# JuliaParallel/DistributedArrays.jl

Measured on NVIDIA H100. Metric: GB/s for map! and sum on Float32 DArray, higher is better.
Workload: dtype f32

## Files before the change

distributedarrays.jl_b200/_broadcast.py:

```python
from __future__ import annotations

import ctypes as C
import struct
from typing import Callable, List, Optional, Sequence, Tuple

import numpy as np

from builtins import any as builtins_any

from . import _lib
from ._darray import B200Array, DArray, dab_dtype, darray, makelocal
from .layout import shape_of
from .runtime import close_remote_reads, open_remote_reads, runtime

_RANK = {"bool": 0, "i32": 1, "i64": 2, "i128": 3, "f32": 4, "f64": 5}


class _TagTypes(dict):

    def __missing__(self, tag):
        raise _lib.UnsupportedError(_lib.ERR_UNSUPPORTED, f"values of type {tag} have no array element type on the GPU backend "
                                    "(Int128 is served as the value type of mapreduce(f, op, d) only)")


_NPT = _TagTypes({"bool": np.dtype(np.bool_), "i32": np.dtype(np.int32), "i64": np.dtype(np.int64), "f32": np.dtype(np.float32),
                  "f64": np.dtype(np.float64), "c64": np.dtype(np.complex64), "c128": np.dtype(np.complex128)})
# ... 426 lines not shown


def jl_max(a, b):
    return binop("max", Expr.wrap(a), Expr.wrap(b))


def jl_min(a, b):
    return binop("min", Expr.wrap(a), Expr.wrap(b))


def mod(a, b):
    return binop("mod", Expr.wrap(a), Expr.wrap(b))


def rem(a, b):
    return binop("rem", Expr.wrap(a), Expr.wrap(b))


def trace(f: Callable, arg_tags: Sequence[str]) -> Expr:
    syms = [Expr("arg", (), t, k) for k, t in enumerate(arg_tags)]
    return Expr.wrap(f(*syms))


_FN2 = {"add": "jl_add", "sub": "jl_sub", "mul": "jl_mul", "div": "jl_div", "rem": "jl_rem", "mod": "jl_mod", "idiv": "jl_idiv",
        "max": "jl_max", "min": "jl_min", "pow": "jl_pow", "and": "jl_and", "or": "jl_or", "xor": "jl_xor", "lt": "jl_lt", "le": "jl_le",
        "gt": "jl_gt", "ge": "jl_ge", "eq": "jl_eq", "ne": "jl_ne", "x_shl": "jl_x_shl", "x_shr": "jl_x_shr"}
_FN2.update({"m_copysign": "jl_m_copysign", "m_powi": "jl_m_powi"})
_FN2.update({"m_" + c: "jl_m_" + c for c in ("lt", "le", "gt", "ge", "eq", "ne")})


def _lit(jt: str, v) -> str:
    if jt == "f32":
        return "__int_as_float((int)0x%08x)" % struct.unpack("<I", struct.pack("<f", float(v)))[0]
    if jt == "f64":
        return "__longlong_as_double((long long)0x%016xULL)" % struct.unpack("<Q", struct.pack("<d", float(v)))[0]
    if is_ctag(jt):
        z = complex(v)
        return "%s(%s, %s)" % (_CT[jt], _lit(_COMP[jt], z.real), _lit(_COMP[jt], z.imag))
    if jt == "i32":
        return "((int)%d)" % int(v)
    if jt == "i64":
        return "((long long)%dLL)" % int(v)
    if jt == "i128":
        v = int(v) % (1 << 128)
        return "((i128)(((u128)0x%016xULL << 64) | (u128)0x%016xULL))" % (v >> 64, v & ((1 << 64) - 1))
    return "true" if v else "false"
# ... 75 lines not shown
        groups.append((o, ext))
    if not groups:
        groups = [(1, [1] * len(shapes))]
    return tuple(g[0] for g in groups), [tuple(g[1][k] for g in groups) for k in range(len(shapes))]


def _dense_strides(shape):
    s, out = 1, []
    for d in shape:
        out.append(s)
        s *= int(d)
    return out


class LocalArg:

    def __init__(self, arr: Optional[B200Array] = None, scalar=None, tag: str = "f64", temp: bool = False):
        self.arr, self.scalar, self.tag, self.temp = arr, scalar, tag, temp


def run_local(rt, expr: Expr, out: B200Array, largs: List[LocalArg]):
    n = out.size
    if n == 0:
        return
    out_tag = tag_of(out.dtype)
    full = [a for a in largs if a.arr is not None]
    same = all(a.arr.shape == out.shape or a.arr.size == n and _squeeze(a.arr.shape) == _squeeze(out.shape) for a in full)
    ctx = rt.ctx
    code = dab_dtype(out.dtype)
    rt.last_kernel = "fixed"
    cplx = uses_complex(expr) or builtins_any(is_ctag(a.tag) for a in largs)
    if same and not cplx and expr.jt == out_tag and out_tag != "bool":
        x0 = largs[0] if largs and largs[0].arr is not None and largs[0].tag == out_tag else None
        if x0 is not None and all(_only_arg0(expr)):
            ab = match_affine(expr)
            if ab is not None:
                a = np.asarray(ab[0], dtype=out.dtype)
                b = np.asarray(ab[1], dtype=out.dtype)
                _lib.call("dab_affine", ctx, code, C.c_void_p(out.ptr), C.c_void_p(x0.arr.ptr), C.c_void_p(a.ctypes.data),
                          C.c_void_p(b.ctypes.data), n)
                rt.last_kernel = "dab_affine"
                return
            if expr.op in _UN and _is_arg(expr.args[0], 0):
                _lib.call("dab_unary", ctx, code, _UN[expr.op], C.c_void_p(out.ptr), C.c_void_p(x0.arr.ptr), n)
                return
            if _is_arg(expr, 0):
                _lib.call("dab_unary", ctx, code, _lib.MAP_ID, C.c_void_p(out.ptr), C.c_void_p(x0.arr.ptr), n)
                return
        if expr.op in _BIN and len(expr.args) == 2 and not (expr.op == "div" and out_tag[0] != "f"):
            l, r = expr.args
            la = largs[l.val] if l.op == "arg" else None
            ra = largs[r.val] if r.op == "arg" else None

            def arr_ok(e, a):
                return e.op == "arg" and a is not None and a.arr is not None and a.tag == out_tag

            def sc_val(e, a):
                if e.op == "const" and e.jt == out_tag:
                    return e.val
                if e.op == "arg" and a is not None and a.arr is None and a.tag == out_tag:
                    return a.scalar
                return None

            if arr_ok(l, la) and arr_ok(r, ra):
                _lib.call("dab_binary", ctx, code, _BIN[expr.op], C.c_void_p(out.ptr), C.c_void_p(la.arr.ptr), C.c_void_p(ra.arr.ptr), n)
# ... 120 lines not shown
            out.append((lo, hi))
        else:
            out.append((1, s))
    return tuple(out)


def _localise(rt, a, I, pid) -> LocalArg:
    if isinstance(a, DArray):
        view = _bcview(a.dims, I)
        arr = makelocal(a, view, pid)
        return LocalArg(arr, None, tag_of(a.dtype), temp=arr is not a.chunks.get(pid))
    if isinstance(a, np.ndarray) and a.ndim > 0:
        view = _bcview(a.shape, I)
        sl = a[tuple(slice(lo - 1, hi) for lo, hi in view)]
        return LocalArg(B200Array.from_numpy(rt, sl), None, tag_of(a.dtype), temp=True)
    e = Expr.wrap(a.item() if isinstance(a, np.ndarray) else a)
    return LocalArg(None, e.val, e.jt)


def _remote_args(dest_layout, args) -> List[DArray]:
    return [a for a in args if isinstance(a, DArray) and not (a.layout.pids == dest_layout.pids and a.layout.indices == dest_layout.indices)]


def _broadcast_chunks(dest: DArray, expr: Expr, args) -> DArray:
    rt = dest.rt
    fenced = open_remote_reads(rt, _remote_args(dest.layout, args), "host")
    for pid, out in dest.chunks.items():
        I = dest.layout.localindices(pid)
        largs = [_localise(rt, a, I, pid) for a in args]
        run_local(rt, expr, out, largs)
        for la in largs:
            if la.temp and la.arr is not None:
                la.arr.free()
    close_remote_reads(rt, fenced, "host")
    return dest


def _materialise_views(args):
    from ._darray import SubDArray
    out, temps = [], []
    for a in args:
        if isinstance(a, SubDArray):
            a = a.to_darray()
            temps.append(a)
        out.append(a)
    return out, temps


def broadcast_into(dest: DArray, f: Callable, *args) -> DArray:
    args, _views = _materialise_views(args)
    try:
        return _broadcast_into(dest, f, *args)
    finally:
        for v in _views:
            v.close()


def _broadcast_into(dest: DArray, f: Callable, *args) -> DArray:
    shapes = [a.dims if isinstance(a, DArray) else (a.shape if isinstance(a, np.ndarray) else ()) for a in args]
    for shp in shapes:
        for k, s in enumerate(shp):
            want = dest.dims[k] if k < len(dest.dims) else 1
            if s != 1 and s != want:
                raise _lib.DimensionMismatch(_lib.ERR_DIM_MISMATCH, f"destination axes {dest.dims} are not compatible with source axes {tuple(shp)}")
    expr = trace(f, [_arg_tag(a) for a in args])
    return _broadcast_chunks(dest, expr, args)


def broadcast(f: Callable, *args, rt=None) -> DArray:
    args, _views = _materialise_views(args)
    try:
        return _broadcast(f, *args, rt=rt)
    finally:
        for v in _views:
            v.close()


def _broadcast(f: Callable, *args, rt=None) -> DArray:
    rt = rt or next((a.rt for a in args if isinstance(a, DArray)), None) or runtime()
    shapes = [a.dims if isinstance(a, DArray) else (a.shape if isinstance(a, np.ndarray) else ()) for a in args]
    dims = _bc_shape(shapes)
    expr = trace(f, [_arg_tag(a) for a in args])
    out_dt = _NPT[expr.jt]
    dest = darray(lambda I: B200Array.empty(rt, shape_of(I), out_dt), dims, dtype=out_dt, rt=rt)
    return _broadcast_chunks(dest, expr, args)


def copy(d: DArray) -> DArray:
    from ._darray import similar
    return _broadcast_into(similar(d), lambda x: x, d)


deepcopy = copy


def drandn(dims, procs=None, dist=None, dtype=np.float64, seed: int = 1234, rt=None) -> DArray:
    from ._darray import component_dtype, drand
    dt = np.dtype(dtype)
    if dt.kind == "c":
        ct = component_dtype(dt)
        re = drandn(dims, procs, dist, dtype=ct, seed=seed, rt=rt)
        im = drandn(dims, procs, dist, dtype=ct, seed=seed + 2, rt=rt)
        from ._darray import darray_like
        out = darray_like(lambda I: B200Array.empty(re.rt, shape_of(I), dt), re, dtype=dt)
        _broadcast_into(out, lambda a, b: complex_(0.7071067811865476 * a, 0.7071067811865476 * b), re, im)
# ... 55 lines not shown
```

distributedarrays.jl_b200/_darray.py:

```python
from __future__ import annotations

import ctypes as C
import itertools
import weakref
from typing import Callable, Dict, List, Optional, Sequence, Tuple

import numpy as np

from . import _lib
from .layout import Layout, Range, default_procs, layout_from_chunk_shapes, make_layout, rlen, shape_of, slab_plan
from .runtime import Runtime, close_remote_reads, open_remote_reads, runtime

_DT = {np.dtype(np.float32): _lib.F32, np.dtype(np.float64): _lib.F64, np.dtype(np.int32): _lib.I32,
       np.dtype(np.int64): _lib.I64, np.dtype(np.bool_): _lib.U8,
       np.dtype(np.complex64): _lib.C64, np.dtype(np.complex128): _lib.C128}
_NP = {_lib.F32: np.dtype(np.float32), _lib.F64: np.dtype(np.float64), _lib.I32: np.dtype(np.int32),
       _lib.I64: np.dtype(np.int64), _lib.U8: np.dtype(np.bool_), _lib.C64: np.dtype(np.complex64), _lib.C128: np.dtype(np.complex128)}


def dab_dtype(dt) -> int:
    dt = np.dtype(dt)
    if dt not in _DT:
        raise _lib.UnsupportedError(_lib.ERR_UNSUPPORTED, f"element type {dt} is not served by the GPU backend (no host fallback)")
    return _DT[dt]


# ... 22 lines not shown
    __slots__ = ("rt", "ptr", "shape", "dtype", "_own", "_keep", "_temp")

    def __init__(self, rt: Runtime, ptr: int, shape: Sequence[int], dtype, own: bool = True, keep=None, temp: bool = False):
        self.rt, self.ptr, self.shape, self.dtype = rt, int(ptr), tuple(int(s) for s in shape), np.dtype(dtype)
        self._own, self._keep, self._temp = own, keep, temp

    @classmethod
    def empty(cls, rt: Runtime, shape: Sequence[int], dtype, temp: bool = False) -> "B200Array":
        dtype = np.dtype(dtype)
        n = int(np.prod(shape)) if len(shape) else 1
        ptr = rt.alloc_temp(n * dtype.itemsize) if temp else rt.alloc(n * dtype.itemsize)
        return cls(rt, ptr, shape, dtype, temp=temp)

    @classmethod
    def from_numpy(cls, rt: Runtime, a: np.ndarray) -> "B200Array":
        a = np.asarray(a)
        dab_dtype(a.dtype)
        out = cls.empty(rt, a.shape, a.dtype)
        out.copy_from_host(a)
        return out

    @property
    def size(self) -> int:
        return int(np.prod(self.shape)) if len(self.shape) else 1

    @property
    def nbytes(self) -> int:
        return self.size * self.dtype.itemsize

    @property
    def ndim(self) -> int:
        return len(self.shape)

    def copy_from_host(self, a: np.ndarray, sync: bool = True):
        a = np.asarray(a, dtype=self.dtype)
        if tuple(a.shape) != self.shape:
            raise _lib.DimensionMismatch(_lib.ERR_DIM_MISMATCH, f"host array {a.shape} vs chunk {self.shape}")
        if self.size == 0:
            return
        if not a.flags.f_contiguous:
            if a.ndim == 2 and a.strides[0] == a.itemsize and a.strides[1] > 0:
                _lib.call("dab_h2d_2d", self.rt.ctx, C.c_void_p(self.ptr), a.shape[0] * a.itemsize, C.c_void_p(a.ctypes.data),
                          a.strides[1], a.shape[0] * a.itemsize, a.shape[1])
                if sync:
                    self.rt.sync()
                return
            a = np.asfortranarray(a)
# ... 657 lines not shown
```

distributedarrays.jl_b200/_mapreduce.py:

```python
from __future__ import annotations

import builtins
import ctypes as C
import operator
from typing import Callable, Dict, Optional, Sequence, Tuple

import numpy as np

from . import _lib
from ._broadcast import Expr, broadcast, is_ctag, tag_of, trace, _NPT
from ._darray import B200Array, DArray, component_dtype, dab_dtype, is_complex, np_dtype
from .layout import Layout, collapse_for_region, ravel, shape_of, unravel
from .runtime import close_remote_reads, exchange_stacks, fence, grouped_exchange, open_remote_reads

_OPS = {"+": _lib.SUM, "add": _lib.SUM, "sum": _lib.SUM, "*": _lib.PROD, "mul": _lib.PROD, "prod": _lib.PROD, "max": _lib.MAX,
        "min": _lib.MIN}
_OPF = {operator.add: _lib.SUM, operator.mul: _lib.PROD, builtins.max: _lib.MAX, builtins.min: _lib.MIN, np.add: _lib.SUM,
        np.multiply: _lib.PROD, np.maximum: _lib.MAX, np.minimum: _lib.MIN}


def _op_code(op) -> int:
    if isinstance(op, str) and op in _OPS:
        return _OPS[op]
    if op in _OPF:
        return _OPF[op]
    raise _lib.UnsupportedError(_lib.ERR_UNSUPPORTED, f"reduction operator {op!r} is not served by a kernel (no host fallback)")
# ... 25 lines not shown
    if e.op in _CMPMAP:
        l, r = e.args

        def unpromote(side, const):
            if side.op == "convert" and side.args[0].op == "arg" and side.args[0].jt == tag and const.op == "const":
                c = const.val
                if tag == "f32" and const.jt == "f64" and float(np.float32(c)) == c:
                    return side.args[0], Expr("const", (), tag, c)
                if tag in ("i32", "i64") and const.jt in ("i64",) and side.jt == "i64":
                    return side.args[0], Expr("const", (), tag, c) if -2**31 <= c < 2**31 or tag == "i64" else (side, const)
            return side, const

        l, r = unpromote(l, r)
        r, l = unpromote(r, l)
        if l.op == "arg" and r.op == "const" and l.jt == tag:
            return _CMPMAP[e.op], np.asarray(r.val, dtype=np.dtype(dtype)), e
        if r.op == "arg" and l.op == "const" and r.jt == tag:
            return _CMPMAP[_FLIP[e.op]], np.asarray(l.val, dtype=np.dtype(dtype)), e
    if e.op == "isnan" and e.args[0].op == "arg":
        return _lib.MAP_ISNAN, None, e
    return None, None, e


def _result_dtype(dtype, op: int, mapc: int) -> np.dtype:
    out = C.c_int32()
    _lib.check(_lib.lib().dab_reduce_result_dtype(dab_dtype(dtype), op, mapc, C.byref(out)))
    return np.dtype(np.int64) if out.value == _lib.I64 else np_dtype(out.value)




def _gather_slots(d: DArray, launch: Callable[[int, B200Array, int], None]) -> np.ndarray:
    rt = d.rt
    wpr = rt.workers_per_rank
    slots = B200Array.empty(rt, (16 * wpr,), np.uint8, temp=True)
    try:
        for pid, ch in d.chunks.items():
            launch(pid, ch, slots.ptr + 16 * ((pid - 1) % wpr))
        if rt.world > 1:
            allslots = B200Array.empty(rt, (16 * wpr * rt.world,), np.uint8, temp=True)
            _lib.call("dab_allgather", rt.ctx, C.c_void_p(slots.ptr), C.c_void_p(allslots.ptr), 16 * wpr)
            host = allslots.to_numpy()
            allslots.free()
        else:
            host = slots.to_numpy()
    finally:
# ... 109 lines not shown
    return (res, vals) if return_partials else res


def _mapreduce_all(f, op, d: DArray, return_partials: bool = False, others: Sequence = ()):
    opc = op if isinstance(op, int) else _op_code(op)
    if others:
        expr = trace(f, [tag_of(d.dtype)] + [_arg_tag_of(a) for a in others])
        return _mapreduce_expr(expr, opc, d, others, return_partials)
    mapc, param, expr = classify_map(f, d.dtype)
    if is_complex(d.dtype) and mapc is not None and not _complex_served(opc, mapc):
        if mapc == _lib.MAP_ID and opc in (_lib.MAX, _lib.MIN):
            raise TypeError(f"MethodError: no method matching isless(::{d.dtype}, ::{d.dtype}) -- complex numbers are not ordered")
        mapc = None
        if expr is None:
            expr = trace(lambda z: z, [tag_of(d.dtype)])
    if mapc is None:
        return _mapreduce_expr(expr, opc, d, (), return_partials)
    _check_nonempty(d, opc)
    rt = d.rt
    pp = C.c_void_p(param.ctypes.data) if param is not None else None
    rdt = _result_dtype(d.dtype, opc, mapc)
    if rt.workers_per_rank == 1 and d.layout.pids == rt.workers() and not return_partials:
        ch = d.chunks[rt.myid()]
        out = np.zeros(2, dtype=np.uint64)
        _lib.call("dab_mapreduce_all", rt.ctx, dab_dtype(d.dtype), opc, mapc, pp, C.c_void_p(ch.ptr), ch.size, C.c_void_p(out.ctypes.data))
        return out.view(np.uint8)[:rdt.itemsize].view(rdt)[0]
    code = dab_dtype(d.dtype)
    host = _gather_slots(d, lambda pid, ch, slot: _lib.call("dab_reduce", rt.ctx, code, opc, mapc, pp, C.c_void_p(ch.ptr), ch.size, C.c_void_p(slot)))
    res, vals = _fold(host, d.layout.pids, rdt, opc)
    return (res, vals) if return_partials else res


def _complex_served(opc: int, mapc: int) -> bool:
    out = C.c_int32()
    return _lib.lib().dab_reduce_result_dtype(_lib.C64, opc, mapc, C.byref(out)) == _lib.OK


def _arg_tag_of(a) -> str:
    from ._broadcast import _arg_tag
    return _arg_tag(a)


def reduce(op, d: DArray, dims=None, init=None):
    return mapreduce(None, op, d, dims=dims, init=init)


def mapreduce(f: Optional[Callable], op, d: DArray, *ds, dims=None, init=None, _partials: bool = False):
    from ._darray import SubDArray
    if isinstance(d, Expr):
# ... 403 lines not shown
```

distributedarrays.jl_b200/csrc/dab_comm.cu:

```cuda
#include <dlfcn.h>
#include <nccl.h>

#include "dab_common.cuh"
#include "dab_scalar_ops.cuh"

namespace {

struct NcclApi {
    void* handle = nullptr;
    ncclResult_t (*GetUniqueId)(ncclUniqueId*) = nullptr;
    ncclResult_t (*CommInitRank)(ncclComm_t*, int, ncclUniqueId, int) = nullptr;
    ncclResult_t (*CommDestroy)(ncclComm_t) = nullptr;
    ncclResult_t (*AllGather)(const void*, void*, size_t, ncclDataType_t, ncclComm_t, cudaStream_t) = nullptr;
    ncclResult_t (*AllReduce)(const void*, void*, size_t, ncclDataType_t, ncclRedOp_t, ncclComm_t, cudaStream_t) = nullptr;
    ncclResult_t (*Send)(const void*, size_t, ncclDataType_t, int, ncclComm_t, cudaStream_t) = nullptr;
    ncclResult_t (*Recv)(void*, size_t, ncclDataType_t, int, ncclComm_t, cudaStream_t) = nullptr;
    ncclResult_t (*GroupStart)() = nullptr;
    ncclResult_t (*GroupEnd)() = nullptr;
    const char* (*GetErrorString)(ncclResult_t) = nullptr;
    const char* (*GetLastError)(ncclComm_t) = nullptr;
    bool ok = false;
    char why[256] = "";
};

// ... 67 lines not shown
    while (*mine < seq) {
        if ((++spins & 1023u) == 0 && dab_globaltimer_ns() - t0 > timeout_ns) {
            host_status[0] = 1ull;
            __threadfence_system();
            break;
        }
    }
    __threadfence_system();
}

template <typename T>
__global__ void __launch_bounds__(256) accumulate_stack_kernel(T* __restrict__ y, size_t n, T beta, int beta_mode, T alpha, int alpha_one,
                                                              const T* __restrict__ stack, size_t stride, int count) {
    for (size_t i = (size_t)blockIdx.x * 256 + threadIdx.x; i < n; i += (size_t)gridDim.x * 256) {
        T v = beta_mode == 0 ? T(0) : (beta_mode == 1 ? y[i] : jl::mul(y[i], beta));
        for (int j = 0; j < count; ++j) {
            const T r = stack[(size_t)j * stride + i];
            v = jl::add(v, alpha_one ? r : jl::mul(alpha, r));
        }
        y[i] = v;
    }
}

}

extern "C" {

int32_t dab_comm_unique_id(void* id128) {
    NEED_NCCL(nullptr);
    if (!id128) return dab_fail(nullptr, DAB_ERR_ARG, "null id");
    static_assert(sizeof(ncclUniqueId) == 128, "ncclUniqueId is 128 bytes");
    ncclUniqueId id;
    DAB_NCCL(nullptr, api.GetUniqueId(&id));
    memcpy(id128, &id, 128);
    return DAB_OK;
}

int32_t dab_comm_init_rank(dab_ctx* ctx, const void* id128, int32_t rank, int32_t nranks) {
    DAB_ENTER(ctx);
    NEED_NCCL(ctx);
    DAB_REQUIRE(ctx, id128 && nranks >= 1 && rank >= 0 && rank < nranks && nranks <= DAB_MAX_RANKS, DAB_ERR_ARG,
                "dab_comm_init_rank: bad rank %d / nranks %d", rank, nranks);
    DAB_REQUIRE(ctx, !ctx->comm, DAB_ERR_ARG, "communicator already initialised");
    ncclUniqueId id;
    memcpy(&id, id128, 128);
    ncclComm_t comm;
// ... 72 lines not shown
int32_t dab_recv(dab_ctx* ctx, void* recv_dev, size_t nbytes, int32_t peer) {
    DAB_ENTER(ctx);
    NEED_COMM(ctx);
    DAB_NCCL(ctx, api.Recv(recv_dev, nbytes, ncclInt8, peer, (ncclComm_t)ctx->comm, ctx->stream));
    return DAB_OK;
}

int32_t dab_mapreduce_all(dab_ctx* ctx, int32_t dtype, int32_t op, int32_t map, const void* map_param, const void* x, size_t n,
                          void* out_host) {
    DAB_ENTER_NOFLUSH(ctx);
    int32_t rdt;
    if (!out_host || op == DAB_EXTREMA || dab_reduce_result_dtype(dtype, op, map, &rdt) != DAB_OK) {
        DAB_FLUSH(ctx);
        DAB_REQUIRE(ctx, out_host, DAB_ERR_ARG, "dab_mapreduce_all: null out");
        if (op == DAB_EXTREMA) return dab_fail(ctx, DAB_ERR_UNSUPPORTED, "dab_mapreduce_all: extrema combines through dab_reduce + dab_allgather");
        return dab_fail(ctx, DAB_ERR_ARG, "bad dtype/op");
    }
    const bool cplx = rdt == DAB_C64 || rdt == DAB_C128;
    if ((ctx->mbox_ranks > 1 || !ctx->comm || ctx->nranks == 1) && n > 0 && !cplx) {
        ctx->fuse_op = op;
        int32_t st = dab_reduce(ctx, dtype, op, map, map_param, x, n, ctx->result_slot);
        ctx->fuse_op = -1;
        if (st != DAB_OK) return st;
        DAB_CUDA(ctx, cudaStreamSynchronize(ctx->stream));
        const volatile unsigned long long* h = (const volatile unsigned long long*)ctx->host_slot;
        if (h[1] != 0) return dab_fail(ctx, DAB_ERR_NCCL, "fused combine timed out waiting for a peer's chunk result (did every rank call?)");
        unsigned long long bits = h[0];
        memset(out_host, 0, 8);
        memcpy(out_host, &bits, dab_dtype_size(rdt));
        return DAB_OK;
    }
    if (cplx && ctx->mbox_ranks > 1 && !ctx->comm) {
        DAB_FLUSH(ctx);
        return dab_fail(ctx, DAB_ERR_UNSUPPORTED, "dab_mapreduce_all: a complex result across %d ranks needs the NCCL communicator "
                        "(the mailbox combine carries 8-byte results)", ctx->mbox_ranks);
    }
    int32_t st = dab_reduce(ctx, dtype, op, map, map_param, x, n, ctx->result_slot);
    if (st != DAB_OK) return st;
    const int P = ctx->comm ? ctx->nranks : 1;
    const void* src = ctx->result_slot;
    if (P > 1) {
        NEED_COMM(ctx);
        DAB_NCCL(ctx, api.AllGather(ctx->result_slot, ctx->gather_slots, 16, ncclInt8, (ncclComm_t)ctx->comm, ctx->stream));
        ctx->launches++;
        src = ctx->gather_slots;
    }
    DAB_CUDA(ctx, cudaMemcpyAsync(ctx->host_slot, src, (size_t)P * 16, cudaMemcpyDeviceToHost, ctx->stream));
    DAB_CUDA(ctx, cudaStreamSynchronize(ctx->stream));
// ... 136 lines not shown
```

distributedarrays.jl_b200/csrc/dab_common.cuh:

```cuda
#pragma once
#include <cuda_runtime.h>

#include <cstdint>
#include <cstdio>
#include <cstring>

#include "../../include/dab200.h"

#define DAB_MAX_REDUCE_BLOCKS 262144
#define DAB_SLOT_BYTES 64
#define DAB_MAX_RANKS 64

struct dab_pending_affine {
    int active;
    int32_t dtype;
    void* y;
    const void* x;
    size_t n;
    unsigned char a[8], b[8];
};

struct dab_ctx {
    int device;
    int sm_count;
    cudaStream_t stream;
    void* block_partials;
    unsigned int* counter;
    void* result_slot;
    void* gather_slots;
    void* host_slot;
    void* dim_scratch;
    size_t dim_scratch_bytes;
    uint64_t launches;
    void* comm;
    int rank, nranks;
    void* mailbox;
    void** peer_mbox_dev;
    void* peer_mbox_host[DAB_MAX_RANKS];
    int mbox_ranks;
    unsigned long long mbox_seq;
    unsigned long long barrier_seq;
    int fuse_op;
    struct dab_alloc_cache* cache;
    void* sort_dev;
    size_t sort_dev_bytes;
    void* stage[2];
    cudaEvent_t stage_ev[2];
    void* sort_host;
    unsigned long long sort_epoch;
    void* scan_dev;
    size_t scan_dev_bytes;
    unsigned long long scan_epoch;
    unsigned long long scan_tickets;
    void* scan_scratch;
    size_t scan_scratch_bytes;
    long long opt_combine_timeout_ms;
    long long opt_gemm_kc;
    int opt_gemm_rawhi;
    int opt_gemm_simt;
    int opt_gemv_phase;
    int opt_gemv_t_cols;
    int opt_gemv_t_waves;
    int opt_spmv_group;
    int opt_ew_tma;
// ... 43 lines not shown

#define DAB_LAUNCHED(ctx)                          \
    do {                                           \
        (ctx)->launches++;                         \
        DAB_CUDA((ctx), cudaGetLastError());       \
    } while (0)

static inline size_t dab_dtype_size(int32_t dt) {
    switch (dt) {
        case DAB_F32: return 4;
        case DAB_F64: return 8;
        case DAB_I32: return 4;
        case DAB_I64: return 8;
        case DAB_U8: return 1;
        case DAB_C64: return 8;
        case DAB_C128: return 16;
        default: return 0;
    }
}

#define DAB_MBOX_SLOT 32
#define DAB_MBOX_BARRIER_OFFSET (2 * DAB_MAX_RANKS * DAB_MBOX_SLOT)
#define DAB_MBOX_BYTES (DAB_MBOX_BARRIER_OFFSET + DAB_MAX_RANKS * 8)
struct FusedComm {
    void* const* peers;
    void* host_out;
    unsigned long long seq;
    unsigned long long timeout_ns;
    int rank, nranks, op;
};

__device__ __forceinline__ unsigned long long dab_globaltimer_ns() {
    unsigned long long t;
    asm volatile("mov.u64 %0, %globaltimer;" : "=l"(t));
    return t;
}
__device__ __forceinline__ int4 ld_stream(const int4* p) { return __ldcs(p); }
__device__ __forceinline__ void st_stream(int4* p, int4 v) { __stcs(p, v); }

template <typename T>
struct alignas(16) Pack {
    static constexpr int N = 16 / sizeof(T);
    T v[N];
};

template <typename T>
struct alignas(2 * sizeof(T)) Cplx {
    T re, im;
};

template <typename T>
__device__ __forceinline__ Pack<T> as_pack(int4 r) {
    Pack<T> p;
    memcpy(&p, &r, 16);
    return p;
}
template <typename T>
__device__ __forceinline__ int4 as_int4(const Pack<T>& p) {
// ... 26 lines not shown
```

distributedarrays.jl_b200/csrc/dab_core.cu:

```cuda
#include <cstdarg>
#include <cstdlib>
#include <map>
#include <mutex>
#include <new>
#include <thread>
#include <unordered_map>

#include "dab_common.cuh"

thread_local char dab_tls_err[512] = "";

struct dab_alloc_cache {
    std::unordered_map<void*, size_t> live;
    std::multimap<size_t, void*> free_blocks;
    size_t cached_bytes = 0;
    static constexpr size_t kMaxBlock = 16ull << 30;
    static constexpr size_t kMaxCached = 32ull << 30;
};

int dab_resident_ctas(const void* kernel, int threads) {
    static std::mutex mu;
    static std::unordered_map<const void*, int> cache;
    std::lock_guard<std::mutex> lk(mu);
    auto it = cache.find(kernel);
// ... 85 lines not shown
        }                                                                   \
    } while (0)
    INIT_CUDA(cudaSetDevice(device));
    cudaDeviceProp prop;
    INIT_CUDA(cudaGetDeviceProperties(&prop, device));
    if (prop.major != 9 || prop.minor != 0) {
        delete ctx;
        return dab_fail(nullptr, DAB_ERR_UNSUPPORTED, "device %d is sm_%d%d; libdab200 is built for sm_90a only", device,
                        prop.major, prop.minor);
    }
    ctx->sm_count = prop.multiProcessorCount;
    INIT_CUDA(cudaStreamCreateWithFlags(&ctx->stream, cudaStreamNonBlocking));
    {
        cudaMemPool_t pool;
        INIT_CUDA(cudaDeviceGetDefaultMemPool(&pool, device));
        unsigned long long keep = ~0ull;
        INIT_CUDA(cudaMemPoolSetAttribute(pool, cudaMemPoolAttrReleaseThreshold, &keep));
    }
    INIT_CUDA(cudaMalloc(&ctx->block_partials, ((size_t)DAB_MAX_REDUCE_BLOCKS + DAB_MAX_REDUCE_BLOCKS / 256 + 16) * 16));
    INIT_CUDA(cudaMalloc((void**)&ctx->counter, (DAB_MAX_REDUCE_BLOCKS / 256 + 16) * 4));
    INIT_CUDA(cudaMemsetAsync(ctx->counter, 0, (DAB_MAX_REDUCE_BLOCKS / 256 + 16) * 4, ctx->stream));
    INIT_CUDA(cudaMalloc(&ctx->result_slot, DAB_SLOT_BYTES));
    INIT_CUDA(cudaMalloc(&ctx->gather_slots, (size_t)DAB_MAX_RANKS * 16));
    INIT_CUDA(cudaHostAlloc(&ctx->host_slot, (size_t)(DAB_MAX_RANKS + 2) * 16, cudaHostAllocDefault));
    INIT_CUDA(cudaStreamSynchronize(ctx->stream));
    memset(ctx->host_slot, 0, (size_t)(DAB_MAX_RANKS + 2) * 16);
#undef INIT_CUDA
    *out = ctx;
    return DAB_OK;
}

int32_t dab_comm_destroy(dab_ctx* ctx);
int32_t dab_mailbox_detach(dab_ctx* ctx);

int32_t dab_shutdown(dab_ctx* ctx) {
    if (!ctx) return DAB_OK;
    cudaSetDevice(ctx->device);
    const int32_t st = dab_flush_pending(ctx);
    cudaStreamSynchronize(ctx->stream);
    if (ctx->comm) dab_comm_destroy(ctx);
    cudaFree(ctx->block_partials);
    cudaFree(ctx->counter);
    cudaFree(ctx->result_slot);
    cudaFree(ctx->gather_slots);
    if (ctx->dim_scratch) cudaFree(ctx->dim_scratch);
    if (ctx->sort_dev) cudaFree(ctx->sort_dev);
    if (ctx->scan_dev) cudaFree(ctx->scan_dev);
    if (ctx->scan_scratch) cudaFree(ctx->scan_scratch);
    if (ctx->sort_host) cudaFreeHost(ctx->sort_host);
// ... 381 lines not shown
```

distributedarrays.jl_b200/csrc/dab_reduce.cu:

```cuda
#include <type_traits>

#include <cmath>

#include "dab_reduce_traits.cuh"

namespace {

constexpr int RD_UNROLL = 4;

struct NoStore {
    template <typename T>
    __device__ __forceinline__ void vec(Pack<T>&, size_t) const {}
    template <typename T>
    __device__ __forceinline__ T scalar(T v, size_t) const { return v; }
};
template <typename T>
struct AffineStore {
    AffineF<T> f;
    T* y;
    int4* yv;
    __device__ __forceinline__ void vec(Pack<T>& p, size_t i) const {
#pragma unroll
        for (int k = 0; k < Pack<T>::N; ++k) p.v[k] = f(p.v[k]);
        st_stream(yv + i, as_int4(p));
// ... 100 lines not shown
        is_last = (ticket == ngroups - 1);
    }
    __syncthreads();
    if (!is_last) return;
    __threadfence();
    A fin = R::identity();
    for (unsigned int i = threadIdx.x; i < ngroups; i += RD_THREADS) fin = R::comb(fin, gpartials[i]);
    fin = block_reduce<R>(fin, smem);
    if (threadIdx.x == 0) {
        *counter = 0;
        if constexpr (std::is_arithmetic<A>::value) {
            Out res;
            if (finalize_mode == 1) res = (Out)(fin == (A)n_for_all);
            else if (finalize_mode == 2) res = (Out)(fin != (A)0);
            else res = (Out)fin;
            memcpy(out, &res, sizeof(Out));
            if (sizeof(Out) < 8) memset((char*)out + sizeof(Out), 0, 8 - sizeof(Out));
            A wide = fin;
            memcpy((char*)out + 8, &wide, sizeof(A));
            if (sizeof(A) < 8) memset((char*)out + 8 + sizeof(A), 0, 8 - sizeof(A));
            if (fc.host_out && fc.nranks <= 1) {
                unsigned long long bits = 0;
                memcpy(&bits, &res, sizeof(Out));
                volatile unsigned long long* h = reinterpret_cast<volatile unsigned long long*>(fc.host_out);
                h[0] = bits;
                h[1] = 0ull;
                __threadfence_system();
            }
        } else if constexpr (is_cplx<Out>::value) {
            using CT = decltype(Out::re);
            const Out res{(CT)fin.re, (CT)fin.im};
            memset(out, 0, 16);
            memcpy(out, &res, sizeof(Out));
        } else {
            memset(out, 0, 16);
            memcpy(out, &fin, sizeof(A));
        }
    }
    if constexpr (!std::is_arithmetic<Out>::value) return;
    else {
    if (fc.nranks <= 1) return;
    __shared__ unsigned long long pay[2];
    __shared__ unsigned long long got[DAB_MAX_RANKS];
    __shared__ int timed_out;
    if (threadIdx.x == 0) {
        memcpy(&pay[0], out, 8);
        memcpy(&pay[1], (char*)out + 8, 8);
        timed_out = 0;
    }
    __syncthreads();
// ... 16 lines not shown
            }
        }
        __threadfence_system();
        got[threadIdx.x] = src[0];
    }
    __syncthreads();
    if (threadIdx.x == 0) {
        Out a;
        memcpy(&a, &got[0], sizeof(Out));
        for (int j = 1; j < fc.nranks; ++j) {
            Out b;
            memcpy(&b, &got[j], sizeof(Out));
            switch (fc.op) {
                case DAB_SUM: case DAB_COUNT: a = jl::add(a, b); break;
                case DAB_PROD: a = jl::mul(a, b); break;
                case DAB_MAX: a = jl::max(a, b); break;
                case DAB_MIN: a = jl::min(a, b); break;
                case DAB_ALL: a = (Out)(a != (Out)0 && b != (Out)0); break;
                default: a = (Out)(a != (Out)0 || b != (Out)0); break;
            }
        }
        unsigned long long bits = 0;
        memcpy(&bits, &a, sizeof(Out));
        volatile unsigned long long* h = reinterpret_cast<volatile unsigned long long*>(fc.host_out);
        h[0] = bits;
        h[1] = (unsigned long long)timed_out;
        __threadfence_system();
    }
    }
}

template <typename T, typename Map, typename R, typename Out, typename St = NoStore>
int32_t launch_reduce(dab_ctx* ctx, const T* x, size_t n, Map map, void* out, int finalize_mode, St st = St()) {
    constexpr int VPT = 16 / sizeof(T);
    size_t head = ((16 - ((uintptr_t)x & 15)) & 15) / sizeof(T);
    if (head > n) head = n;
    if constexpr (!std::is_same<St, NoStore>::value) st.yv = reinterpret_cast<int4*>(st.y + head);
    size_t tiles = (n - head) / ((size_t)VPT * RD_THREADS * RD_UNROLL);
    size_t k = 2;
    if ((tiles + k - 1) / k > (size_t)DAB_MAX_REDUCE_BLOCKS) k = (tiles + DAB_MAX_REDUCE_BLOCKS - 1) / DAB_MAX_REDUCE_BLOCKS;
    size_t grid = (tiles + k - 1) / k;
    if (grid < 1) grid = 1;
    FusedComm fc;
    memset(&fc, 0, sizeof(fc));
    if (ctx->fuse_op >= 0 && ctx->mbox_ranks > 1) {
        fc.peers = ctx->peer_mbox_dev;
        fc.host_out = ctx->host_slot;
        fc.seq = ++ctx->mbox_seq;
        fc.timeout_ns = (unsigned long long)ctx->opt_combine_timeout_ms * 1000000ull;
        fc.rank = ctx->rank;
        fc.nranks = ctx->mbox_ranks;
        fc.op = ctx->fuse_op;
    } else if (ctx->fuse_op >= 0) {
        fc.host_out = ctx->host_slot;
        fc.nranks = 1;
        fc.op = ctx->fuse_op;
    }
    reduce_kernel<T, Map, R, Out, St><<<(unsigned)grid, RD_THREADS, 0, ctx->stream>>>(x, n, head, map, (typename R::A*)ctx->block_partials,
                                                                                      ctx->counter, out, finalize_mode, (long long)n, (int)k, fc, st);
    DAB_LAUNCHED(ctx);
    return DAB_OK;
}

template <typename T>
using ResultOfSum = typename std::conditional<std::is_floating_point<T>::value, T, long long>::type;

template <typename T, int FN>
int32_t reduce_arith(dab_ctx* ctx, int32_t op, const T* x, size_t n, void* out) {
    MapF<T, FN> map{(T)0};
    switch (op) {
        case DAB_SUM: return launch_reduce<T, MapF<T, FN>, SumTraits<T>, ResultOfSum<T>>(ctx, x, n, map, out, 0);
        case DAB_PROD: return launch_reduce<T, MapF<T, FN>, ProdTraits<T>, ResultOfSum<T>>(ctx, x, n, map, out, 0);
        case DAB_MAX: return launch_reduce<T, MapF<T, FN>, MaxTraits<T>, T>(ctx, x, n, map, out, 0);
        case DAB_MIN: return launch_reduce<T, MapF<T, FN>, MinTraits<T>, T>(ctx, x, n, map, out, 0);
        case DAB_EXTREMA:
            if constexpr (FN == DAB_MAP_ID) return launch_reduce<T, ExtMapF<T>, ExtremaTraits<T>, Pair<T>>(ctx, x, n, ExtMapF<T>{(T)0}, out, 0);
            else return dab_fail(ctx, DAB_ERR_UNSUPPORTED, "extrema with a map is not served (no host fallback)");
// ... 367 lines not shown
```

Measured before the change: 4284.

## Cache traced broadcast plans and replay affine launches; spin-wait on fused reduce completion

Caches traced expressions keyed by function code, closures and scalar globals. For repeated map! calls it stores a replay plan of dab_affine launch arguments, checked against weak references and chunk pointers, so later calls skip tracing and chunk localisation. The fused single-rank sum now has the kernel post a completion sequence word to pinned host memory, and the host spins on it with periodic stream queries instead of calling cudaStreamSynchronize. Smaller host-side trims (math.prod, an lru_cache on the result dtype, a ctypes output buffer) cut Python overhead further, at the cost of cache invalidation complexity and CPU busy-waiting.

Result: faster. 4350 (median of 6 runs) (+1.5%).

```diff
diff --git a/distributedarrays.jl_b200/_broadcast.py b/distributedarrays.jl_b200/_broadcast.py
--- a/distributedarrays.jl_b200/_broadcast.py
+++ b/distributedarrays.jl_b200/_broadcast.py
@@ -1,7 +1,10 @@
 from __future__ import annotations
 
+import builtins as _builtins
 import ctypes as C
 import struct
+import types
+import weakref
 from typing import Callable, List, Optional, Sequence, Tuple
 
 import numpy as np
@@ -474,6 +477,90 @@
     return Expr.wrap(f(*syms))
 
 
+_TRACE_CACHE: dict = {}
+_TRACE_CACHE_MAX = 256
+_UNBOUND = object()
+
+
+_SCALAR_KIND: dict = {bool: 0, int: 0, float: 1, complex: 2}
+_CODE_OK: dict = {}
+
+
+def _scalar_key(v):
+    t = type(v)
+    kind = _SCALAR_KIND.get(t)
+    if kind is None:
+        kind = _SCALAR_KIND[t] = 3 if issubclass(t, (np.bool_, np.number)) else -1
+    if kind == 3:
+        return t, v.tobytes()
+    if kind == 0:
+        return t, v
+    if kind == 1:
+        return t, struct.pack("<d", v)
+    if kind == 2:
+        return t, struct.pack("<dd", v.real, v.imag)
+    return None
+
+
+def _trace_key(f: Callable, arg_tags: Sequence[str]):
+    if type(f) is not types.FunctionType:
+        return None
+    code = f.__code__
+    ok = _CODE_OK.get(code)
+    if ok is None:
+        ok = _CODE_OK[code] = not builtins_any(isinstance(c, types.CodeType) for c in code.co_consts)
+    if not ok:
+        return None
+    keys = [code, tuple(arg_tags)]
+    if f.__closure__:
+        for c in f.__closure__:
+            try:
+                k = _scalar_key(c.cell_contents)
+            except ValueError:
+                return None
+            if k is None:
+                return None
+            keys.append(k)
+    for v in f.__defaults__ or ():
+        k = _scalar_key(v)
+        if k is None:
+            return None
+        keys.append(k)
+    keys.append(None)
+    if f.__kwdefaults__:
+        for name, v in sorted(f.__kwdefaults__.items()):
+            k = _scalar_key(v)
+            if k is None:
+                return None
+            keys.append((name, k))
+    keys.append(None)
+    if code.co_names:
+        g = f.__globals__
+        for name in code.co_names:
+            v = g[name] if name in g else _builtins.__dict__.get(name, _UNBOUND)
+            if v is _UNBOUND:
+                keys.append(None)
+                continue
+            k = _scalar_key(v)
+            if k is None:
+                return None
+            keys.append(k)
+    return tuple(keys)
+
+
+def trace_cached(f: Callable, arg_tags: Sequence[str]) -> Expr:
+    key = _trace_key(f, arg_tags)
+    if key is None:
+        return trace(f, arg_tags)
+    e = _TRACE_CACHE.get(key)
+    if e is None:
+        e = trace(f, arg_tags)
+        if len(_TRACE_CACHE) >= _TRACE_CACHE_MAX:
+            del _TRACE_CACHE[next(iter(_TRACE_CACHE))]
+        _TRACE_CACHE[key] = e
+    return e
+
+
 _FN2 = {"add": "jl_add", "sub": "jl_sub", "mul": "jl_mul", "div": "jl_div", "rem": "jl_rem", "mod": "jl_mod", "idiv": "jl_idiv",
         "max": "jl_max", "min": "jl_min", "pow": "jl_pow", "and": "jl_and", "or": "jl_or", "xor": "jl_xor", "lt": "jl_lt", "le": "jl_le",
         "gt": "jl_gt", "ge": "jl_ge", "eq": "jl_eq", "ne": "jl_ne", "x_shl": "jl_x_shl", "x_shr": "jl_x_shr"}
@@ -595,7 +682,7 @@
 def run_local(rt, expr: Expr, out: B200Array, largs: List[LocalArg]):
     n = out.size
     if n == 0:
-        return
+        return _NO_LAUNCH
     out_tag = tag_of(out.dtype)
     full = [a for a in largs if a.arr is not None]
     same = all(a.arr.shape == out.shape or a.arr.size == n and _squeeze(a.arr.shape) == _squeeze(out.shape) for a in full)
@@ -610,10 +697,10 @@
             if ab is not None:
                 a = np.asarray(ab[0], dtype=out.dtype)
                 b = np.asarray(ab[1], dtype=out.dtype)
-                _lib.call("dab_affine", ctx, code, C.c_void_p(out.ptr), C.c_void_p(x0.arr.ptr), C.c_void_p(a.ctypes.data),
-                          C.c_void_p(b.ctypes.data), n)
+                call = (code, C.c_void_p(out.ptr), C.c_void_p(x0.arr.ptr), C.c_void_p(a.ctypes.data), C.c_void_p(b.ctypes.data), n, a, b)
+                _lib.call("dab_affine", ctx, *call[:6])
                 rt.last_kernel = "dab_affine"
-                return
+                return call
             if expr.op in _UN and _is_arg(expr.args[0], 0):
                 _lib.call("dab_unary", ctx, code, _UN[expr.op], C.c_void_p(out.ptr), C.c_void_p(x0.arr.ptr), n)
                 return
@@ -780,18 +867,73 @@
     return [a for a in args if isinstance(a, DArray) and not (a.layout.pids == dest_layout.pids and a.layout.indices == dest_layout.indices)]
 
 
-def _broadcast_chunks(dest: DArray, expr: Expr, args) -> DArray:
+def _broadcast_chunks(dest: DArray, expr: Expr, args, calls: Optional[list] = None) -> DArray:
     rt = dest.rt
     fenced = open_remote_reads(rt, _remote_args(dest.layout, args), "host")
+    replayable = calls is not None and not fenced
     for pid, out in dest.chunks.items():
         I = dest.layout.localindices(pid)
         largs = [_localise(rt, a, I, pid) for a in args]
-        run_local(rt, expr, out, largs)
+        call = run_local(rt, expr, out, largs)
+        if replayable:
+            if call is None or builtins_any(la.temp for la in largs):
+                replayable = False
+            elif call is not _NO_LAUNCH:
+                calls.append(call)
         for la in largs:
             if la.temp and la.arr is not None:
                 la.arr.free()
     close_remote_reads(rt, fenced, "host")
+    if calls is not None and not replayable:
+        calls.clear()
     return dest
+
+
+_NO_LAUNCH = ()
+_PLANS: dict = {}
+_PLANS_MAX = 64
+
+
+class _AffinePlan:
+    __slots__ = ("expr", "refs", "chunks", "calls")
+
+    def __init__(self, expr, arrays, calls):
+        self.expr = expr
+        self.refs = [weakref.ref(d) for d in arrays]
+        self.chunks = [(d.layout, len(d.chunks), [(pid, ch, ch.ptr) for pid, ch in d.chunks.items()]) for d in arrays]
+        self.calls = calls
+
+    def valid(self, expr, arrays) -> bool:
+        if self.expr is not expr or len(arrays) != len(self.refs):
+            return False
+        for ref, d, (layout, n, snap) in zip(self.refs, arrays, self.chunks):
+            if ref() is not d or d.layout is not layout or len(d.chunks) != n:
+                return False
+            chunks = d.chunks
+            for pid, ch, ptr in snap:
+                if chunks.get(pid) is not ch or ch.ptr != ptr:
+                    return False
+        return True
+
+
+def _plan_key(f, dest, args):
+    tags, keys = [], [id(dest)]
+    for a in args:
+        if type(a) is DArray:
+            tags.append(tag_of(a.dtype))
+            keys.append(id(a))
+        else:
+            k = _scalar_key(a)
+            if k is None:
+                return None, None
+            tags.append(Expr.wrap(a).jt)
+            keys.append(k)
+    tk = _trace_key(f, tags)
+    expr = _TRACE_CACHE.get(tk) if tk is not None else None
+    if expr is None:
+        return None, None
+    keys.append(id(expr))
+    return expr, tuple(keys)
 
 
 def _materialise_views(args):
@@ -806,6 +948,15 @@
 
 
 def broadcast_into(dest: DArray, f: Callable, *args) -> DArray:
+    if type(dest) is DArray:
+        expr, key = _plan_key(f, dest, args)
+        plan = _PLANS.get(key) if key is not None else None
+        if plan is not None and plan.valid(expr, [dest] + [a for a in args if type(a) is DArray]):
+            rt = dest.rt
+            for call in plan.calls:
+                _lib.call("dab_affine", rt.ctx, *call[:6])
+            rt.last_kernel = "dab_affine"
+            return dest
     args, _views = _materialise_views(args)
     try:
         return _broadcast_into(dest, f, *args)
@@ -821,8 +972,18 @@
             want = dest.dims[k] if k < len(dest.dims) else 1
             if s != 1 and s != want:
                 raise _lib.DimensionMismatch(_lib.ERR_DIM_MISMATCH, f"destination axes {dest.dims} are not compatible with source axes {tuple(shp)}")
-    expr = trace(f, [_arg_tag(a) for a in args])
-    return _broadcast_chunks(dest, expr, args)
+    expr = trace_cached(f, [_arg_tag(a) for a in args])
+    if type(dest) is not DArray:
+        return _broadcast_chunks(dest, expr, args)
+    calls: list = []
+    _broadcast_chunks(dest, expr, args, calls)
+    if calls:
+        pexpr, key = _plan_key(f, dest, args)
+        if key is not None and pexpr is expr:
+            if len(_PLANS) >= _PLANS_MAX:
+                del _PLANS[next(iter(_PLANS))]
+            _PLANS[key] = _AffinePlan(expr, [dest] + [a for a in args if type(a) is DArray], calls)
+    return dest
 
 
 def broadcast(f: Callable, *args, rt=None) -> DArray:
@@ -838,7 +999,7 @@
     rt = rt or next((a.rt for a in args if isinstance(a, DArray)), None) or runtime()
     shapes = [a.dims if isinstance(a, DArray) else (a.shape if isinstance(a, np.ndarray) else ()) for a in args]
     dims = _bc_shape(shapes)
-    expr = trace(f, [_arg_tag(a) for a in args])
+    expr = trace_cached(f, [_arg_tag(a) for a in args])
     out_dt = _NPT[expr.jt]
     dest = darray(lambda I: B200Array.empty(rt, shape_of(I), out_dt), dims, dtype=out_dt, rt=rt)
     return _broadcast_chunks(dest, expr, args)
diff --git a/distributedarrays.jl_b200/_darray.py b/distributedarrays.jl_b200/_darray.py
--- a/distributedarrays.jl_b200/_darray.py
+++ b/distributedarrays.jl_b200/_darray.py
@@ -2,6 +2,7 @@
 
 import ctypes as C
 import itertools
+import math
 import weakref
 from typing import Callable, Dict, List, Optional, Sequence, Tuple
 
@@ -70,7 +71,7 @@
 
     @property
     def size(self) -> int:
-        return int(np.prod(self.shape)) if len(self.shape) else 1
+        return math.prod(self.shape)
 
     @property
     def nbytes(self) -> int:
diff --git a/distributedarrays.jl_b200/_mapreduce.py b/distributedarrays.jl_b200/_mapreduce.py
--- a/distributedarrays.jl_b200/_mapreduce.py
+++ b/distributedarrays.jl_b200/_mapreduce.py
@@ -2,6 +2,7 @@
 
 import builtins
 import ctypes as C
+import functools
 import operator
 from typing import Callable, Dict, Optional, Sequence, Tuple
 
@@ -73,6 +74,7 @@
     return None, None, e
 
 
+@functools.lru_cache(maxsize=256)
 def _result_dtype(dtype, op: int, mapc: int) -> np.dtype:
     out = C.c_int32()
     _lib.check(_lib.lib().dab_reduce_result_dtype(dab_dtype(dtype), op, mapc, C.byref(out)))
@@ -228,9 +230,9 @@
     rdt = _result_dtype(d.dtype, opc, mapc)
     if rt.workers_per_rank == 1 and d.layout.pids == rt.workers() and not return_partials:
         ch = d.chunks[rt.myid()]
-        out = np.zeros(2, dtype=np.uint64)
-        _lib.call("dab_mapreduce_all", rt.ctx, dab_dtype(d.dtype), opc, mapc, pp, C.c_void_p(ch.ptr), ch.size, C.c_void_p(out.ctypes.data))
-        return out.view(np.uint8)[:rdt.itemsize].view(rdt)[0]
+        out = (C.c_uint64 * 2)()
+        _lib.call("dab_mapreduce_all", rt.ctx, dab_dtype(d.dtype), opc, mapc, pp, C.c_void_p(ch.ptr), ch.size, out)
+        return np.frombuffer(out, dtype=rdt, count=1)[0]
     code = dab_dtype(d.dtype)
     host = _gather_slots(d, lambda pid, ch, slot: _lib.call("dab_reduce", rt.ctx, code, opc, mapc, pp, C.c_void_p(ch.ptr), ch.size, C.c_void_p(slot)))
     res, vals = _fold(host, d.layout.pids, rdt, opc)
diff --git a/distributedarrays.jl_b200/csrc/dab_comm.cu b/distributedarrays.jl_b200/csrc/dab_comm.cu
--- a/distributedarrays.jl_b200/csrc/dab_comm.cu
+++ b/distributedarrays.jl_b200/csrc/dab_comm.cu
@@ -113,6 +113,32 @@
     }
 }
 
+inline void cpu_relax() {
+#if defined(__x86_64__) || defined(__i386__)
+    __builtin_ia32_pause();
+#elif defined(__aarch64__)
+    asm volatile("yield" ::: "memory");
+#endif
+}
+
+int32_t wait_done(dab_ctx* ctx) {
+    const unsigned long long want = ctx->done_seq;
+    unsigned long long* word = (unsigned long long*)((char*)ctx->host_slot + DAB_HOST_DONE_OFFSET) + 2;
+    for (unsigned int spins = 1;; ++spins) {
+        if (__atomic_load_n(word, __ATOMIC_ACQUIRE) == want) return DAB_OK;
+        if ((spins & 255u) == 0) {
+            const cudaError_t e = cudaStreamQuery(ctx->stream);
+            if (e == cudaSuccess) {
+                if (__atomic_load_n(word, __ATOMIC_ACQUIRE) == want) return DAB_OK;
+                return dab_fail(ctx, DAB_ERR_CUDA, "dab_mapreduce_all: the fused reduce finished without posting its result "
+                                "(completion word %llu, expected %llu)", __atomic_load_n(word, __ATOMIC_ACQUIRE), want);
+            }
+            if (e != cudaErrorNotReady) return dab_fail_cuda(ctx, e, "cudaStreamQuery (fused reduce)", __FILE__, __LINE__);
+        }
+        cpu_relax();
+    }
+}
+
 }
 
 extern "C" {
@@ -231,8 +257,9 @@
         int32_t st = dab_reduce(ctx, dtype, op, map, map_param, x, n, ctx->result_slot);
         ctx->fuse_op = -1;
         if (st != DAB_OK) return st;
-        DAB_CUDA(ctx, cudaStreamSynchronize(ctx->stream));
-        const volatile unsigned long long* h = (const volatile unsigned long long*)ctx->host_slot;
+        st = wait_done(ctx);
+        if (st != DAB_OK) return st;
+        const volatile unsigned long long* h = (const volatile unsigned long long*)((char*)ctx->host_slot + DAB_HOST_DONE_OFFSET);
         if (h[1] != 0) return dab_fail(ctx, DAB_ERR_NCCL, "fused combine timed out waiting for a peer's chunk result (did every rank call?)");
         unsigned long long bits = h[0];
         memset(out_host, 0, 8);
diff --git a/distributedarrays.jl_b200/csrc/dab_common.cuh b/distributedarrays.jl_b200/csrc/dab_common.cuh
--- a/distributedarrays.jl_b200/csrc/dab_common.cuh
+++ b/distributedarrays.jl_b200/csrc/dab_common.cuh
@@ -40,6 +40,7 @@
     int mbox_ranks;
     unsigned long long mbox_seq;
     unsigned long long barrier_seq;
+    unsigned long long done_seq;
     int fuse_op;
     struct dab_alloc_cache* cache;
     void* sort_dev;
@@ -129,9 +130,12 @@
 #define DAB_MBOX_SLOT 32
 #define DAB_MBOX_BARRIER_OFFSET (2 * DAB_MAX_RANKS * DAB_MBOX_SLOT)
 #define DAB_MBOX_BYTES (DAB_MBOX_BARRIER_OFFSET + DAB_MAX_RANKS * 8)
+#define DAB_HOST_DONE_OFFSET ((DAB_MAX_RANKS + 2) * 16)
+#define DAB_HOST_SLOT_BYTES (DAB_HOST_DONE_OFFSET + 32)
 struct FusedComm {
     void* const* peers;
     void* host_out;
+    unsigned long long done_seq;
     unsigned long long seq;
     unsigned long long timeout_ns;
     int rank, nranks, op;
@@ -141,6 +145,13 @@
     unsigned long long t;
     asm volatile("mov.u64 %0, %globaltimer;" : "=l"(t));
     return t;
+}
+__device__ __forceinline__ void dab_post_done(const FusedComm& fc, unsigned long long bits, unsigned long long status) {
+    volatile unsigned long long* h = reinterpret_cast<volatile unsigned long long*>(fc.host_out);
+    h[0] = bits;
+    h[1] = status;
+    __threadfence_system();
+    h[2] = fc.done_seq;
 }
 __device__ __forceinline__ int4 ld_stream(const int4* p) { return __ldcs(p); }
 __device__ __forceinline__ void st_stream(int4* p, int4 v) { __stcs(p, v); }
diff --git a/distributedarrays.jl_b200/csrc/dab_core.cu b/distributedarrays.jl_b200/csrc/dab_core.cu
--- a/distributedarrays.jl_b200/csrc/dab_core.cu
+++ b/distributedarrays.jl_b200/csrc/dab_core.cu
@@ -131,9 +131,9 @@
     INIT_CUDA(cudaMemsetAsync(ctx->counter, 0, (DAB_MAX_REDUCE_BLOCKS / 256 + 16) * 4, ctx->stream));
     INIT_CUDA(cudaMalloc(&ctx->result_slot, DAB_SLOT_BYTES));
     INIT_CUDA(cudaMalloc(&ctx->gather_slots, (size_t)DAB_MAX_RANKS * 16));
-    INIT_CUDA(cudaHostAlloc(&ctx->host_slot, (size_t)(DAB_MAX_RANKS + 2) * 16, cudaHostAllocDefault));
+    INIT_CUDA(cudaHostAlloc(&ctx->host_slot, DAB_HOST_SLOT_BYTES, cudaHostAllocDefault));
     INIT_CUDA(cudaStreamSynchronize(ctx->stream));
-    memset(ctx->host_slot, 0, (size_t)(DAB_MAX_RANKS + 2) * 16);
+    memset(ctx->host_slot, 0, DAB_HOST_SLOT_BYTES);
 #undef INIT_CUDA
     *out = ctx;
     return DAB_OK;
diff --git a/distributedarrays.jl_b200/csrc/dab_reduce.cu b/distributedarrays.jl_b200/csrc/dab_reduce.cu
--- a/distributedarrays.jl_b200/csrc/dab_reduce.cu
+++ b/distributedarrays.jl_b200/csrc/dab_reduce.cu
@@ -146,10 +146,7 @@
             if (fc.host_out && fc.nranks <= 1) {
                 unsigned long long bits = 0;
                 memcpy(&bits, &res, sizeof(Out));
-                volatile unsigned long long* h = reinterpret_cast<volatile unsigned long long*>(fc.host_out);
-                h[0] = bits;
-                h[1] = 0ull;
-                __threadfence_system();
+                dab_post_done(fc, bits, 0ull);
             }
         } else if constexpr (is_cplx<Out>::value) {
             using CT = decltype(Out::re);
@@ -212,10 +209,7 @@
         }
         unsigned long long bits = 0;
         memcpy(&bits, &a, sizeof(Out));
-        volatile unsigned long long* h = reinterpret_cast<volatile unsigned long long*>(fc.host_out);
-        h[0] = bits;
-        h[1] = (unsigned long long)timed_out;
-        __threadfence_system();
+        dab_post_done(fc, bits, (unsigned long long)timed_out);
     }
     }
 }
@@ -233,16 +227,18 @@
     if (grid < 1) grid = 1;
     FusedComm fc;
     memset(&fc, 0, sizeof(fc));
+    if (ctx->fuse_op >= 0) {
+        fc.host_out = (char*)ctx->host_slot + DAB_HOST_DONE_OFFSET;
+        fc.done_seq = ++ctx->done_seq;
+    }
     if (ctx->fuse_op >= 0 && ctx->mbox_ranks > 1) {
         fc.peers = ctx->peer_mbox_dev;
-        fc.host_out = ctx->host_slot;
         fc.seq = ++ctx->mbox_seq;
         fc.timeout_ns = (unsigned long long)ctx->opt_combine_timeout_ms * 1000000ull;
         fc.rank = ctx->rank;
         fc.nranks = ctx->mbox_ranks;
         fc.op = ctx->fuse_op;
     } else if (ctx->fuse_op >= 0) {
-        fc.host_out = ctx->host_slot;
         fc.nranks = 1;
         fc.op = ctx->fuse_op;
     }
```
